# hamza1030/stereo_matching_cuda

Hardware: AMD Instinct MI355X
Metric: disparity MPix/s (stereo pair -> L+R disparity + occlusion-filled map) (higher is better)
Workload: dtype f32; 1 GPU; kitti 1242x375 D=192 seeded synthetic pair (seed 20150101); width=1242, height=375, disparities=192, slices_in_flight=192, walker_launches_per_call=1

## Files before the change

stereo_matching_cuda_amd/csrc/smx_agg_v5.hip:

```cpp
#include <stdlib.h>
#include <string.h>

#include <type_traits>

#include "smx_agg_dev.h"
#include "smx_agg_v5.h"
#include "smx_v5_diag.h"

namespace smx {
namespace v5 {
using namespace aggdev;

constexpr int R = 9, HW = 2 * R + 1;
constexpr int SWU = HW * L;
constexpr int SW = (SWU + 3) / 4 * 4;
static_assert(OWS == HW * (L - 1) && SWU == OWS + HW && CPW * L <= 64 && CPW * NS1 >= HW, "strip geometry");
constexpr int RD = 20;
static_assert(RD % BH == 0 && RD >= HW + 1, "ring");
static_assert(L == 9, "the shipped form: seven combs of nine lanes per comb wave");
constexpr int NX = 2;
constexpr int NWAVE = 2 * NS1 + NX, NT = 64 * NWAVE;
constexpr int WPE = 4;
constexpr int NT1 = 3, NT2 = 2;
enum Role { ROLE_S1 = 0, ROLE_S2 = 1, ROLE_SCAN = 2, ROLE_COST = 3 };
// ... 21 lines not shown
    return d;
}

__device__ __forceinline__ f2 div_ca(f2 x, f2 ca) {
    f2 q, e, m;
    asm("v_pk_mul_f32 %0, %1, %2 op_sel_hi:[1,0]" : "=v"(q) : "v"(x), "v"(ca));
    asm("v_pk_fma_f32 %0, %1, %2, %3 op_sel:[0,1,0] op_sel_hi:[1,1,1] neg_lo:[1,0,0] neg_hi:[1,0,0]" : "=v"(e) : "v"(q), "v"(ca), "v"(x));
    asm("v_pk_fma_f32 %0, %1, %2, %3 op_sel_hi:[1,0,1]" : "=v"(m) : "v"(e), "v"(ca), "v"(q));
    return m;
}

__device__ __forceinline__ f2 div_ca_q(f2 x, f2 ca) { f2 q; asm("v_pk_mul_f32 %0, %1, %2 op_sel_hi:[1,0]" : "=v"(q) : "v"(x), "v"(ca)); return q; }
__device__ __forceinline__ f2 div_ca_e(f2 q, f2 x, f2 ca) {
    f2 e;
    asm("v_pk_fma_f32 %0, %1, %2, %3 op_sel:[0,1,0] op_sel_hi:[1,1,1] neg_lo:[1,0,0] neg_hi:[1,0,0]" : "=v"(e) : "v"(q), "v"(ca), "v"(x));
    return e;
}
__device__ __forceinline__ f2 div_ca_m(f2 e, f2 q, f2 ca) { f2 m; asm("v_pk_fma_f32 %0, %1, %2, %3 op_sel_hi:[1,0,1]" : "=v"(m) : "v"(e), "v"(ca), "v"(q)); return m; }

__device__ __forceinline__ unsigned cost_trunc_h2(unsigned q1, unsigned q2, unsigned th2) {
    unsigned d;
    asm("v_pk_add_f16 %0, %1, %2 neg_lo:[0,1] neg_hi:[0,1]" : "=v"(d) : "v"(q1), "v"(q2));
    d &= 0x7fff7fffu;
    asm("v_pk_min_f16 %0, %1, %2" : "=v"(d) : "v"(d), "s"(th2));
    return d;
}
__device__ __forceinline__ float mix_mul_lo(unsigned h2, float s) {
    float r;
    asm("v_fma_mix_f32 %0, %1, %2, 0 op_sel_hi:[1,0,0]" : "=v"(r) : "v"(h2), "s"(s));
    return r;
}
__device__ __forceinline__ float mix_mul_hi(unsigned h2, float s) {
    float r;
    asm("v_fma_mix_f32 %0, %1, %2, 0 op_sel:[1,0,0] op_sel_hi:[1,0,0]" : "=v"(r) : "v"(h2), "s"(s));
    return r;
}
__device__ __forceinline__ float mix_mul_lo_v(unsigned h2, float v) {
    float r;
    asm("v_fma_mix_f32 %0, %1, %2, 0 op_sel_hi:[1,0,0]" : "=v"(r) : "v"(h2), "v"(v));
    return r;
}

__device__ __forceinline__ f2 tile_rd(const float* p) { return (f2){p[0], p[P1]}; }
__device__ __forceinline__ void tile_wr(float* p, f2 v) { p[0] = v.x; p[P1] = v.y; }

template <int FASTK, int QP>
__global__ __launch_bounds__(NT, WPE) void k_v5_walk(Args A) {
    constexpr bool QPERM = QP != 0;
    __shared__ __attribute__((aligned(16))) float tile1[NT1][TILE_F];
    __shared__ __attribute__((aligned(16))) float tile2s[NT2][TILE_F];
    __shared__ float cin1s[2][BH][2];
    __shared__ float rcp_s[RCP_N];
    __shared__ int s_queue[4];
    __shared__ unsigned s_peekn;
    __shared__ unsigned s_seen;
    __shared__ unsigned s_peek[2];
    __shared__ unsigned s_x1;

    const int lane = threadIdx.x & 63;
    const int wave = __builtin_amdgcn_readfirstlane(threadIdx.x >> 6);
    const int tid = 64 * wave + lane;
    const int w = A.w, h = A.h, K = A.K, NI = A.NI, nsv = A.nsv;
    const CostConst cc = A.cc;
    const f2 NZ2 = {-0.0f, -0.0f};
    if (tid < RCP_N) rcp_s[tid] = kRcp.v[tid];

    const bool st2w = wave >= NS1 && wave < 2 * NS1;
    auto comb_il = [&]() { return opaque(lane) % L; };
    auto comb_rho = [&]() {
        const int l = opaque(lane), c = l / L;
        return c < CPW ? CPW * (wave - (st2w ? NS1 : 0)) + c : HW;
    };
    auto comb_jt = [&]() {
        const int rho = comb_rho(), il = comb_il();
        return rho < HW ? HW * il + rho : 0;
    };
    constexpr int NQROW = SW / 4;
    constexpr int NCT = 64;
    constexpr int NRB = 4;
    constexpr int NRBC = 4;
    static_assert(2 * NRBC >= (BH * (SW / 4) + 63) / 64, "two batches");
    constexpr int NCT2 = 0;
    constexpr int NQT = BH * NQROW;
    constexpr int NRQ = (NQT - NCT2 + NCT - 1) / NCT;

    if (tid == 0) {
        s_queue[0] = (int)__hip_atomic_fetch_add((gu32*)A.ticket, 1u, __ATOMIC_RELAXED, __HIP_MEMORY_SCOPE_AGENT);
        s_x1 = 0u; s_peek[0] = 0u; s_peek[1] = 0u; s_peekn = 0u;
    }
    const int P = A.P, q_last = (h + 37) / 10;
    const unsigned fgw4 = ((unsigned)w + 2u * PADX) * 4u, w4 = (unsigned)w * 4u;
    const rsrc_t r_fix = mk_rsrc(A.fix, A.fix_bytes);
    const unsigned recb = (unsigned)(NI + 2) * REC_U * 16u;
    const rsrc_t r_hand = mk_rsrc(A.hand, (size_t)2 * nsv * recb);
    {
        auto item_body = [&](auto ROLEc) {
        constexpr int ROLE = decltype(ROLEc)::value;
        constexpr bool ST2 = ROLE == ROLE_S2, COMB = ROLE <= ROLE_S2;
        int item = 0, k = 0, sv = 0, view = 0, slice = 0, d = 0;
        int base1 = 0;
        int base2 = 0;
        bool pred = false, succ = false;
        bool xedge = false;
        unsigned* myflag = A.flags;
        int o_fg1 = 0, o_fg2 = 0, o_g1p = 0, o_i2p = 0, o_i2b = 0, o_in = 0, o_out = 0;
        rsrc_t r_q = r_fix;
        int q_pitch = 0, q_row0 = 0;
        auto decode = [&](int it) {
            item = it;
            k = it / nsv;
            sv = it - k * nsv;
            view = sv / A.nslices;
            slice = sv - view * A.nslices;
            base1 = OWS * k - 1;
            base2 = OWS * k - R - 1;
            pred = k > 0; succ = k + 1 < K;
            d = A.d0[view] + slice;
            myflag = A.flags + (size_t)sv * K + k;
            o_fg1 = (int)A.o_fg[view]; o_fg2 = (int)A.o_fg[view ^ 1];
            o_g1p = (int)(A.o_g1p[view] + (unsigned)k * (unsigned)(5 * NI) * (CLP * 16u));
            o_i2p = (int)(A.o_i2p[view] + (unsigned)k * (unsigned)NI * (CLP * 16u));
            o_i2b = (int)(A.o_i2p[view] + (unsigned)K * (unsigned)NI * (CLP * 16u) + (unsigned)k * (unsigned)NI * (CLP * 4u));
            o_in = (int)((((unsigned)(k - 1) & 1u) * (unsigned)nsv + (unsigned)sv) * recb);
            o_out = (int)((((unsigned)k & 1u) * (unsigned)nsv + (unsigned)sv) * recb);
            r_q = mk_rsrc(A.q[view] + (size_t)slice * A.q_plane, A.q_plane * 4);
            q_pitch = QPERM ? OWS * 8 : (int)w4; q_row0 = QPERM ? k * ((h + 1) / 2) * (OWS * 8) : 0;
            xedge = base1 < 0 || base1 + SW > w;
        };
        float* tile2 = tile2s[0];
        float (*cin1)[2] = cin1s[0];
        const int jt = comb_jt();
        int xw = 1;
        float rcp_i = 1.0f;
        unsigned vo = OOB;
        unsigned vg = 0;
        bool col_ok = false;
        f2 ca_i = {1.0f, 1.0f};
        uint64_t okmask = 0;
        const bool il0 = comb_il() == 0;
        int jw = 0;
        static_assert(SW + 16 <= P1 && P1 + SW + 16 <= RS, "padding columns behind both planes of a tile row");
        auto lane_consts = [&]() {
            const int il = comb_il();
            const int xo = (ST2 ? base2 - R : base2) + jt;
            col_ok = comb_rho() < HW && xo >= 0 && xo < w && (!ST2 || il >= 1);
            xw = col_ok ? min(w - 1, xo + R) - max(-1, xo - R - 1) : 1;
            rcp_i = rcp_s[HW * xw];
            {
                const int cl = 64 * (wave - (st2w ? NS1 : 0)) + lane;
                vg = (unsigned)cl * (ST2 ? 4u : 16u);
                vo = !col_ok ? OOB : (QPERM ? (unsigned)(k + 1 < K ? (L - 1) * comb_rho() + il - 1 : HW * (il - 1) + comb_rho()) * 8u : (unsigned)xo * 4u);
            }
            ca_i = (f2){rcp_i, (float)(HW * xw)};
            okmask = __builtin_amdgcn_ballot_w64(col_ok);
            jw = (comb_rho() < HW && !(pred && comb_il() == 0)) ? jt : SW + (lane & 15);
        };

        f2 ring[COMB ? RD : 1];
        auto ring_reset = [&]() {
#pragma unroll
            for (int s = 0; s < (COMB ? RD : 1); ++s) ring[s] = (f2){0.0f, 0.0f};
            if constexpr (COMB) ring[ST2 ? 10 : RD - 1] = NZ2;
        };
        ring_reset();
        f4 gr[ROLE == ROLE_S1 ? 2 : 1];
        for (int e = 0; e < (ROLE == ROLE_S1 ? 2 : 1); ++e) gr[e] = (f4){0, 0, 0, 0};
        unsigned gI[ST2 ? BH / 2 : 1];
        f2 r2[ST2 ? BH : 1];
#pragma unroll
        for (int t = 0; t < (ST2 ? BH : 1); ++t) r2[t] = NZ2;
        f4 hreg = {0, 0, 0, 0};
        bool have_pref = false;
        unsigned seen = 0;

        auto cost_unit = [&](int r, int& row, int& col, bool& on) {
            const int u = NCT2 + r * NCT + opaque(lane);
            on = u < NQT;
            const int uc = min(u, NQT - 1);
            row = uc / NQROW;
            col = (uc - row * NQROW) * 4;
        };
        constexpr int CWN = ROLE == ROLE_COST ? NRQ : 1;
        unsigned cw_a1[CWN], cw_a2[CWN], cw_t[CWN], cw_rowb[CWN], cw_m[CWN];
        for (int r = 0; r < CWN; ++r) { cw_a1[r] = 0u; cw_a2[r] = 0u; cw_t[r] = 0u; cw_rowb[r] = 0u; cw_m[r] = 0u; }
        auto cost_consts = [&]() {
          if constexpr (ROLE == ROLE_COST) {
#pragma unroll
            for (int r = 0; r < NRQ; ++r) {
                int row, col; bool on;
                cost_unit(r, row, col, on);
                const unsigned rowb = (unsigned)row * fgw4;
                cw_rowb[r] = (unsigned)opaque((int)rowb);
                cw_a1[r] = (unsigned)opaque((int)((unsigned)(min(max(base1 + col, -PADX), w) + PADX) * 4u + rowb));
                cw_a2[r] = A.src_cost ? (unsigned)opaque((row * w + base1 + col) * 4)
                                      : (unsigned)opaque((int)((unsigned)(min(max(base1 + col + d, -PADX), w) + PADX) * 4u + rowb));
                cw_t[r] = (unsigned)opaque((int)(on ? (unsigned)(row * RS + col) * 4u : (unsigned)SW * 4u));
                unsigned m = 0;
#pragma unroll
                for (int j = 0; j < 4; ++j) m |= (base1 + col + j >= 0 && base1 + col + j < w) ? 1u << j : 0u;
                cw_m[r] = (unsigned)opaque((int)(m | ((unsigned)row << 8)));
            }
          }
        };
        rsrc_t r_c = r_fix;
        unsigned c_max = 0u, c_min1 = 0xffffffffu;
        const unsigned plane4 = (unsigned)(A.cost_plane * 4);
        auto cost_verdict = [&]() {
            if constexpr (ROLE == ROLE_COST) {
                if (A.src_cost && __builtin_amdgcn_ballot_w64(c_max > 0x5d800000u || c_min1 < 0x21800000u - 1u) != 0 && lane == 0)
                    flag_store(A.bad, 1u);
                c_max = 0u; c_min1 = 0xffffffffu;
            }
        };
        auto cost_rsrc = [&]() {
            if constexpr (ROLE == ROLE_COST) {
                if (A.src_cost) r_c = mk_rsrc(A.cost[view] + (size_t)slice * A.cost_plane, A.cost_plane * 4);
            }
        };
        auto cost_lin = [&](int ib, int r, int& linc4, int& sh) {
            const int row = (int)(cw_m[r] >> 8);
            const int e = max(0, BH * ib + row - (h - 1));
            const int lin4 = (int)cw_a2[r] + (BH * ib - e) * (int)w4;
            linc4 = min(max(lin4, 0), (int)plane4 - 16);
            sh = (lin4 - linc4) >> 2;
        };
        u4 cw_ra[CWN], cw_rb[CWN];
// ... 72 lines not shown
                    }
                }
#pragma unroll
                for (int j = 0; j < 4; ++j) ip[j] = mix_mul_lo_v(q1[j], pp[j]);
                if constexpr (EDGE) {
                    const bool rowok = bandb + cw_rowb[r] <= ymaxb;
#pragma unroll
                    for (int j = 0; j < 4; ++j)
                        if (!(rowok && (((cw_m[r] & 0xffu) >> j) & 1u) != 0u)) { pp[j] = -0.0f; ip[j] = -0.0f; }
                }
                *(f4*)(dstb + cw_t[r]) = pp;
                *(f4*)(dstb + cw_t[r] + P1 * 4) = ip;
            }
        };
        auto eval_band_p = [&](int ib, float* dst) {
            static_assert(2 * NRB >= CWN, "two batches");
            auto run = [&](auto EDGEc, auto SRCc) {
                constexpr int NB = decltype(SRCc)::value ? NRBC : NRB;
                cw_issue(ib, std::integral_constant<int, 0>{}, EDGEc, SRCc);
                cw_finish(ib, dst, std::integral_constant<int, 0>{}, EDGEc, SRCc);
                if constexpr (NB < CWN) {
                    cw_issue(ib, std::integral_constant<int, NB>{}, EDGEc, SRCc);
                    cw_finish(ib, dst, std::integral_constant<int, NB>{}, EDGEc, SRCc);
                }
            };
            const bool edge = xedge || BH * ib + BH > h;
            if (A.src_cost) {
                if (edge) run(std::true_type{}, std::true_type{}); else run(std::false_type{}, std::true_type{});
            } else if (edge) run(std::true_type{}, std::false_type{});
            else { V5_MARK("cost begin"); run(std::false_type{}, std::false_type{}); V5_MARK("cost end"); }
        };
        static_assert(BH == 10, "five row pairs per band");
        auto g1_load = [&](int P, auto Sc) {
            if constexpr (ROLE == ROLE_S1) {
                const int Pc = __builtin_amdgcn_readfirstlane(min(max(P, 0), 5 * NI - 1));
                const unsigned vgl = (unsigned)(64 * wave + opaque(lane)) * 16u;
                gr[decltype(Sc)::value] = __builtin_bit_cast(f4, __builtin_amdgcn_raw_buffer_load_b128(r_fix, (int)vgl, o_g1p + Pc * (CLP * 16), 0));
            }
        };
        auto issue_guid = [&](int ib, int yq0) {
            const int ibc = __builtin_amdgcn_readfirstlane(min(max(ib, 0), NI - 1));
            if constexpr (ST2) {
                const u4 a = __builtin_bit_cast(u4, __builtin_amdgcn_raw_buffer_load_b128(r_fix, (int)(vg * 4u), o_i2p + ibc * (CLP * 16), 0));
                gI[0] = a.x; gI[1] = a.y; gI[2] = a.z; gI[3] = a.w;
                gI[4] = ldu(r_fix, vg, o_i2b + ibc * (CLP * 4));
            }
        };

        auto hu_idx = [&]() { return ST2 ? opaque(tid) - 64 * NS1 : opaque(tid); };
        auto fetch_rec = [&](int rec) {
            const int hq = hu_idx();
            hreg = ld16_sc1(r_hand, (unsigned)(o_in + rec * REC_U * 16) + (hq >= 0 && hq < REC_U ? (unsigned)hq * 16u : 0u));
        };
        auto spin_pred = [&](unsigned need) {
            const uint64_t t0 = __builtin_amdgcn_s_memrealtime();
            for (;;) {
                const unsigned f = flag_load(myflag - 1);
                if (f >= need) { s_seen = f; break; }
                __builtin_amdgcn_s_sleep(4);
                if (__builtin_amdgcn_s_memrealtime() - t0 > 200000000ull || flag_load(A.status) != 0u) {
                    flag_store(A.status, 1u + (unsigned)item);
                    s_seen = FLAG_DONE;
                    break;
                }
            }
        };

        auto rowscans = [&](int i1, int i2, float* t1p, float* t2p, float (*cinp)[2], bool pred1, bool pred2) {
            const int sc_l = lane & 31, sc_st = lane >> 5, sc_row = sc_l % BH, sc_comp = sc_l / BH;
            const bool sc_on = sc_l < 2 * BH;
            const int y = sc_st == 0 ? BH * i1 + sc_row : BH * i2 - R + sc_row;
            const bool act = sc_on && y >= 0 && y < h && (sc_st == 0 ? i1 >= 0 : i2 >= 0);
            if (!act) return;
            float* const row = (sc_st == 0 ? t1p : t2p) + sc_row * RS + sc_comp * P1;
            const bool keep = sc_st == 1 && pred2;
            float acc = (sc_st == 0 && pred1) ? cinp[sc_row][sc_comp] : -0.0f;
            f4* const r4 = (f4*)row;
            constexpr int NG = SW / 4;
            constexpr int PF = 4;
            f4 v[PF];
#pragma unroll
            for (int g = 0; g < PF; ++g) v[g] = r4[g];
            f4 xo[2] = {{0, 0, 0, 0}, {0, 0, 0, 0}};
#pragma unroll
            for (int g = 0; g < NG; ++g) {
                const f4 in = v[g % PF];
                if (g + PF < NG) v[g % PF] = r4[g + PF];
                f4& x = xo[g & 1];
                acc = in.x + acc; x.x = acc;
                acc = in.y + acc; x.y = acc;
                acc = in.z + acc; x.z = acc;
                if (g == 4 && keep) acc = in.z;
                acc = in.w + acc; x.w = acc;
                if (g < 5 && keep) { x.x = in.x; x.y = in.y; x.z = in.z; if (g < 4) x.w = in.w; }
                r4[g] = x;
                asm volatile("" :: "v"(xo[(g & 1) ^ 1]));
            }
        };

        auto area_ix = [&](int y) {
            const unsigned yh = min((unsigned)(min(y + R, h - 1) - max(y - R - 1, -1)), (unsigned)HW);
            return (int)__umul24((unsigned)xw, max(yh, 1u));
        };
        auto rcp_pair = [&](int y) {
            const int a0 = area_ix(y), a1 = area_ix(y + 1);
            return (f4){rcp_s[a0], (float)a0, rcp_s[a1], (float)a1};
        };
        f4 rcb = {1.0f, 1.0f, 1.0f, 1.0f};

        unsigned x1_need = 0;
        auto wait_x1 = [&]() {
            for (unsigned spins = 0; __hip_atomic_load(&s_x1, __ATOMIC_RELAXED, __HIP_MEMORY_SCOPE_WORKGROUP) < x1_need; ++spins) {
                __builtin_amdgcn_s_sleep(1);
                if (spins > (1u << 24)) { flag_store(A.status, 1u + (unsigned)item); break; }
            }
            asm volatile("" ::: "memory");
        };
        auto rows1_pair = [&](auto N0c, auto EDGEc, auto BORDERc, auto WAITc, int i, const float* t1, f2& rv) {
            f2 caa = ca_i, cab = ca_i;
            f4 rcn = {1.0f, 1.0f, 1.0f, 1.0f};
            constexpr int N0 = decltype(N0c)::value, T0 = N0 % BH, GS = (N0 / BH + T0 / 2) & 1;
            constexpr bool BORDER = decltype(BORDERc)::value;
            constexpr bool EDGE = decltype(EDGEc)::value || BORDER;
            constexpr int SLa = N0, SLb = N0 + 1, SLPa = (N0 + RD - 1) % RD, S01a = (N0 + 1) % RD, S01b = (N0 + 2) % RD;
            const f2 rvb = tile_rd(t1 + (T0 + 1) * RS + jt);
            const f2 rvn = tile_rd(t1 + (T0 + 2 < BH ? T0 + 2 : T0 + 1) * RS + jt);
            const int ya = BH * i - R + T0;
            if constexpr (decltype(BORDERc)::value) {
                caa = (f2){rcb.x, rcb.y};
                cab = (f2){rcb.z, rcb.w};
                rcn = rcp_pair(ya + 2);
            }
            const f2 old_a = ring[S01a];
            ring[SLa] = rv + ring[SLPa];
            f2 ua = box_bottom(ring[SLa]);
            const f2 sb = rvb + ring[SLa];
            ua = ua - old_a;
            f2 ub = box_bottom(sb);
            ua = box_top(ua, old_a);
            ring[SLb] = sb;
            ub = ub - ring[S01b];
            if constexpr (EDGE) {
                const f2 u0a = ring[SLa] - old_a;
                if (il0 && k == 0) ua = u0a;
            }
            const f2 qa = div_ca_q(ua, caa);
            ub = box_top(ub, ring[S01b]);
            if constexpr (EDGE) {
                const f2 u0b = sb - ring[S01b];
                if (il0 && k == 0) ub = u0b;
            }
            const f2 qb = div_ca_q(ub, cab);
            f2 ma = qa, mb = qb;
            if constexpr (!FASTK) ma = div_ca_m(div_ca_e(qa, ua, caa), qa, caa);
            const f2 ga = {gr[GS].x, gr[GS].y}, gb = {gr[GS].z, gr[GS].w};
            const float mma = ga.x * ma.x;
            if constexpr (!FASTK) mb = div_ca_m(div_ca_e(qb, ub, cab), qb, cab);
            const float ta = ma.y - mma;
            const float mmb = gb.x * mb.x;
            const float aka = 1.0f * ta * ga.y;
            const float tb = mb.y - mmb;
            const float mb2a = 1.0f * ga.x * aka;
            const float akb = 1.0f * tb * gb.y;
            const float bka = 1.0f * ma.x - mb2a;
            const float mb2b = 1.0f * gb.x * akb;
// ... 49 lines not shown
                    tiny = !(amin >= 0x1p-100f);
                } else {
                    float m1, m2;
                    asm("v_min_f32 %0, |%1|, |%2|" : "=v"(m1) : "v"(ua.x), "v"(ua.y));
                    mb = div_ca_m(div_ca_e(qb, ub, cab), qb, cab);
                    asm("v_min_f32 %0, |%1|, |%2|" : "=v"(m2) : "v"(ub.x), "v"(ub.y));
                    tiny = (va && !(m1 >= 0x1p-100f)) || (vb && !(m2 >= 0x1p-100f));
                }
            }
            if (!FASTK && (__builtin_amdgcn_ballot_w64(tiny) & okmask) != 0) {
                asm volatile("; exact-division slow path");
                ma.x = 1.0f * ua.x / caa.y; ma.y = 1.0f * ua.y / caa.y;
                mb.x = 1.0f * ub.x / cab.y; mb.y = 1.0f * ub.y / cab.y;
            }
            const fg_t ip = __builtin_bit_cast(fg_t, gI[T0 / 2]);
            const float tqa = ma.x * (float)ip.x;
            const float tqb = mb.x * (float)ip.y;
            float qva = tqa + ma.y;
            float qvb = tqb + mb.y;
            if constexpr (QPERM) {
                if (va) __builtin_amdgcn_raw_buffer_store_b64((u2){__builtin_bit_cast(unsigned, qva), __builtin_bit_cast(unsigned, qvb)}, r_q, (int)vo, q_row0 + (yq >> 1) * q_pitch, AUX_NT);
            } else {
                if (va) __builtin_amdgcn_raw_buffer_store_b32(__builtin_bit_cast(unsigned, qva), r_q, (int)vo, q_row0 + yq * q_pitch, AUX_NT);
                if (vb) __builtin_amdgcn_raw_buffer_store_b32(__builtin_bit_cast(unsigned, qvb), r_q, (int)vo, q_row0 + (yq + 1) * q_pitch, AUX_NT);
            }
            if constexpr (BORDER) rcb = rcn;
            __builtin_amdgcn_sched_barrier(0);
        };

        auto hand_in = [&](bool halo, const f4 hreg) {
            const int hq = hu_idx();
            if (hq >= 0 && hq < NHU) {
                if (halo) {
                    const int t = hq / 10, j = (hq - 10 * t) * 2;
                    float* dst = tile2 + t * RS + j;
                    dst[0] = hreg.x;
                    dst[P1] = hreg.y;
                    if (j + 1 < HW) { dst[1] = hreg.z; dst[P1 + 1] = hreg.w; }
                }
            } else if (hq >= NHU && hq < REC_U) {
                const int tp = hq - NHU;
                cin1[2 * tp][0] = hreg.x; cin1[2 * tp][1] = hreg.y;
                cin1[2 * tp + 1][0] = hreg.z; cin1[2 * tp + 1][1] = hreg.w;
            }
        };

        float* G1[3] = {tile1[1], tile1[2], tile1[0]};
        float* G2[2] = {tile2s[0], tile2s[1]};
        float (*GC[2])[2] = {cin1s[0], cin1s[1]};
        int g = 0;
        int nf = 0;
        int slf = -2;
        bool ending = false;
        bool f_pred = false;
        bool own = false;
        constexpr int sw = 1;
        int pend_item = 0; bool pend = false;
        int sl2 = 0;
        bool b_pred = false, b_own = false;
        int nxt = 0;

        auto slot_s1 = [&](auto PARc, int sl) {
            constexpr int PAR = decltype(PARc)::value;
            [[maybe_unused]] const int i = g;
            if constexpr (ROLE == ROLE_S1) {
                fetch_rec(min(sl + 2, NI - 1));
                if (sl == -2) {
                    g1_load(0, std::integral_constant<int, 0>{});
                    g1_load(1, std::integral_constant<int, 1>{});
                }
                if (sl >= 0) {
                    const float* const t1 = G1[0];
                    f2 rv = tile_rd(t1 + jt);
                    tile2 = G2[0];
                    V5_STAMP(3);
                    if (sl == 0 && succ && tid < NCU) {
                        const float* p = t1 + 2 * tid * RS + OWS - 1;
                        st16_sc1(r_hand, (unsigned)o_out + (unsigned)(NHU + tid) * 16u, (f4){p[0], p[P1], p[RS], p[RS + P1]});
                    }
                    if (A.prio) __builtin_amdgcn_s_setprio(PRIO_S1);
                    x1_need = (unsigned)NS1 * (unsigned)(g + 1);
                    const bool border = BH * sl - R < R + 1 || BH * sl - R + BH - 1 > h - 1 - R;
                    V5_STAMP(4);
                    __builtin_amdgcn_sched_barrier(0);
#define V5_P1(TT) rows1_pair(std::integral_constant<int, BH * PAR + TT>{}, std::false_type{}, std::false_type{}, std::integral_constant<bool, TT == 0>{}, sl, t1, rv);
#define V5_P1E(TT) rows1_pair(std::integral_constant<int, BH * PAR + TT>{}, std::true_type{}, std::false_type{}, std::integral_constant<bool, TT == 0>{}, sl, t1, rv);
#define V5_P1B(TT) rows1_pair(std::integral_constant<int, BH * PAR + TT>{}, std::true_type{}, std::true_type{}, std::integral_constant<bool, TT == 0>{}, sl, t1, rv);
                    if (border) { rcb = rcp_pair(BH * sl - R); V5_P1B(0) V5_STAMP(6); V5_P1B(2) V5_STAMP(7); V5_P1B(4) V5_STAMP(8); V5_P1B(6) V5_STAMP(9); V5_P1B(8) V5_STAMP(10); }
                    else if (xedge || k == 0) { V5_P1E(0) V5_P1E(2) V5_P1E(4) V5_P1E(6) V5_P1E(8) }
                    else { V5_MARK("s1rows begin"); V5_P1(0) V5_STAMP(6); V5_P1(2) V5_STAMP(7); V5_P1(4) V5_STAMP(8); V5_P1(6) V5_STAMP(9); V5_P1(8) V5_STAMP(10); V5_MARK("s1rows end"); }
#undef V5_P1
#undef V5_P1E
#undef V5_P1B
                    __builtin_amdgcn_s_setprio(0);
                    V5_STAMP(11);
                }
            }
        };
        auto slot_s2 = [&](auto PARc, int sl) {
            constexpr int PAR = decltype(PARc)::value;
            [[maybe_unused]] const int i = g;
            if constexpr (ST2) {
                if (succ && tid == 64 * 2 * NS1 - 1) flag_store(myflag, (unsigned)sl);
                if (A.prio) __builtin_amdgcn_s_setprio(PRIO_S2HEAD);
                V5_MARK("s2head begin");
                const float* const t2 = G2[0];
#pragma unroll
                for (int t = 0; t < BH; ++t) r2[t] = tile_rd(t2 + t * RS + jt);
                const int hq = hu_idx();
                const bool rec_out = succ && hq >= 0 && hq < REC_U;
                f4 hov = {0.0f, 0.0f, 0.0f, 0.0f};
                if (rec_out) {
                    if (hq < NHU) {
                        const int t = hq / 10, j = (hq - 10 * t) * 2;
                        const float* p = t2 + t * RS + OWS + j;
                        hov = (f4){p[0], p[P1], p[1], p[P1 + 1]};
                    } else {
                        const float* p = G1[0] + 2 * (hq - NHU) * RS + OWS - 1;
                        hov = (f4){p[0], p[P1], p[RS], p[RS + P1]};
                    }
                }
                asm volatile("s_waitcnt lgkmcnt(0)" : "+v"(r2[0]), "+v"(r2[1]), "+v"(r2[2]), "+v"(r2[3]), "+v"(r2[4]), "+v"(r2[5]),
                             "+v"(r2[6]), "+v"(r2[7]), "+v"(r2[8]), "+v"(r2[9]), "+v"(hov) :: "memory");
                if (lane == 0) __hip_atomic_fetch_add(&s_x1, 1u, __ATOMIC_RELAXED, __HIP_MEMORY_SCOPE_WORKGROUP);
                if (rec_out) st16_sc1(r_hand, (unsigned)(o_out + sl * REC_U * 16) + (unsigned)hq * 16u, hov);
                if (BH * (sl - 2) - R + BH - 1 >= h) {
#pragma unroll
                    for (int t = 0; t < BH; ++t)
                        if (BH * (sl - 2) - R + t >= h) r2[t] = NZ2;
                }
                V5_MARK("s2head end");
                __builtin_amdgcn_s_setprio(0);
                V5_STAMP(3);
                V5_STAMP(4);
                bool s2_interior = false;
                if (sl >= 2) {
                    const int yq0 = BH * (sl - 2) - 2 * R;
                    const bool border = yq0 < R + 1 || yq0 + BH - 1 > h - 1 - R;
                    s2_interior = !border && sl != q_last;
                    __builtin_amdgcn_sched_barrier(0);
#define V5_P2(TT) rows2_pair(std::integral_constant<int, BH * PAR + TT>{}, std::false_type{}, sl);
#define V5_P2B(TT) rows2_pair(std::integral_constant<int, BH * PAR + TT>{}, std::true_type{}, sl);
                    if (border) { rcb = rcp_pair(yq0); V5_P2B(0) V5_STAMP(6); V5_P2B(2) V5_STAMP(7); V5_P2B(4) V5_STAMP(8); V5_P2B(6) V5_STAMP(9); V5_P2B(8) V5_STAMP(10); }
                    else { V5_MARK("s2rows begin"); V5_P2(0) V5_STAMP(6); V5_P2(2) V5_STAMP(7); V5_P2(4) V5_STAMP(8); V5_P2(6) V5_STAMP(9); V5_P2(8) V5_STAMP(10); V5_MARK("s2rows end"); }
#undef V5_P2
#undef V5_P2B
                }
                issue_guid(sl, BH * (sl - 1) - 2 * R);
                constexpr int KEEP = QPERM ? S2_KEEP - BH / 2 : S2_KEEP;
                if (s2_interior) asm volatile("s_waitcnt vmcnt(%0)" :: "n"(KEEP) : "memory"); else
                drain_vmem();
            }
        };

        auto iter = [&](auto PARc) -> bool {
            wg_barrier();
            [[maybe_unused]] const int i = g;
            V5_STAMP(0); V5_STAMP(1); V5_STAMP(2);
            if constexpr (ROLE >= ROLE_SCAN) { V5_STAMP(3); V5_STAMP(4); }
            if (slf == -2) {
                const int it = s_queue[nf & 3];
                ending = it >= A.nitems;
                if (ending && nf == 0) return true;
                f_pred = !ending && it / nsv > 0;
                seen = nf > 0 ? s_peekn : 0u;
                if constexpr (ROLE == ROLE_COST) {
                    if (own) cost_verdict();
                    own = !ending;
                    if (own) { decode(it); cost_consts(); cost_rsrc(); }
                } else if constexpr (ROLE == ROLE_S1) {
                    own = !ending;
                    if (own) {
                        decode(it); lane_consts(); ring_reset();
                        gr[0] = (f4){0, 0, 0, 0}; gr[1] = (f4){0, 0, 0, 0};
                    }
                } else if constexpr (ROLE == ROLE_SCAN) {
                    b_pred = pred; b_own = own;
                    own = !ending;
                    if (own) decode(it);
                } else {
                    pend_item = it; pend = !ending;
                }
            } else {
                seen = max(seen, s_peek[g & 1]);
            }
            if constexpr (ST2) {
                if (own && sl2 == q_last + 1 && succ && tid == 64 * 2 * NS1 - 1) flag_store(myflag, FLAG_DONE);
                if (slf == sw) {
                    own = pend;
                    sl2 = sw;
                    if (own) {
                        decode(pend_item); lane_consts(); ring_reset();
#pragma unroll
                        for (int t = 0; t < BH; ++t) r2[t] = NZ2;
                    }
                }
            }
            if constexpr (ROLE == ROLE_SCAN) {
                if (A.prio) __builtin_amdgcn_s_setprio(PRIO_SCAN);
                V5_MARK("scan begin");
                const int i1 = own && slf + 1 < NI ? slf + 1 : -1;
                const int i2 = slf == -2 ? (b_own ? P - 3 : -1) : (own ? slf - 1 : -1);
                rowscans(i1, i2, G1[1], G2[1], GC[0], pred, slf == -2 ? b_pred : pred);
                V5_MARK("scan end");
                __builtin_amdgcn_s_setprio(0);
            } else if constexpr (ROLE == ROLE_COST) {
                if (lane == 63) {
                    unsigned pk = 0u;
                    if (own && pred && seen != FLAG_DONE && seen < (unsigned)(slf + 4)) pk = flag_load(myflag - 1);
                    s_peek[(g + 1) & 1] = pk;
                    if (own && slf == P - 6) {
                        nxt = (int)__hip_atomic_fetch_add((gu32*)A.ticket, 1u, __ATOMIC_RELAXED, __HIP_MEMORY_SCOPE_AGENT);
                        s_queue[(nf + 1) & 3] = nxt;
                    }
                    if (own && slf == P - 3) {
                        unsigned pn = 0u;
                        if (nxt < A.nitems) {
                            const int kn = nxt / nsv, svn = nxt - kn * nsv;
                            if (kn > 0) pn = flag_load(A.flags + (size_t)svn * K + kn - 1);
                        }
                        s_peekn = pn;
                    }
                }
                if (A.prio) __builtin_amdgcn_s_setprio(PRIO_COST);
                if (own && slf + 2 < NI) eval_band_p(slf + 2, G1[2]);
                __builtin_amdgcn_s_setprio(0);
            } else if constexpr (ROLE == ROLE_S1) {
                if (own) slot_s1(PARc, slf);
            } else {
                const int sl = sl2;
                if (own && sl >= 1 && sl <= q_last) {
                    slot_s2(PARc, sl);
                } else if (lane == 0) {
                    __hip_atomic_fetch_add(&s_x1, 1u, __ATOMIC_RELAXED, __HIP_MEMORY_SCOPE_WORKGROUP);
                }
            }
            have_pref = f_pred && (seen == FLAG_DONE || seen >= (unsigned)(slf + 3));
            if (f_pred && !have_pref && slf + 2 < NI) {
                if (tid == 0) spin_pred((unsigned)(slf + 3));
                wg_barrier();
                seen = s_seen;
                if constexpr (ROLE == ROLE_S1) {
                    const int hq = hu_idx();
                    const f4 late = ld16_sc1(r_hand, (unsigned)(o_in + min(slf + 2, NI - 1) * REC_U * 16) + (hq >= 0 && hq < REC_U ? (unsigned)hq * 16u : 0u));
                    cin1 = GC[1]; tile2 = G2[0];
                    hand_in(slf >= 0, late);
                }
            } else if constexpr (ROLE == ROLE_S1) {
                V5_MARK("s1handin begin");
                if (own && pred && slf + 2 < NI) { cin1 = GC[1]; tile2 = G2[0]; hand_in(slf >= 0, hreg); }
                V5_MARK("s1handin end");
            }
            if constexpr (ROLE == ROLE_S1) {
                g1_load(slf >= 0 ? 5 * slf + 6 : slf + 2, PARc);
                if (own && slf == 0 && succ) drain_vmem();
            }
            V5_STAMP(5);
            if (ending && slf == 1) return true;
            { float* const t = G1[0]; G1[0] = G1[1]; G1[1] = G1[2]; G1[2] = t; }
            { float* const t = G2[0]; G2[0] = G2[1]; G2[1] = t; }
            { float (*const t)[2] = GC[0]; GC[0] = GC[1]; GC[1] = t; }
            ++g;
            ++sl2;
            return false;
        };
        for (;;) {
            bool done = false;
            for (slf = -2; slf < 2 && !done; slf += 2) {
                done = iter(std::integral_constant<int, 0>{});
                if (!done) { ++slf; done = iter(std::integral_constant<int, 1>{}); --slf; }
            }
            if (done) break;
            for (slf = 2; slf <= P - 3; slf += 2) {
                (void)iter(std::integral_constant<int, 0>{});
                ++slf;
                (void)iter(std::integral_constant<int, 1>{});
                --slf;
            }
            ++nf;
        }
        if constexpr (ROLE == ROLE_COST) { if (own) cost_verdict(); }
        };
        if (wave < NS1) item_body(std::integral_constant<int, ROLE_S1>{});
        else if (wave < 2 * NS1) item_body(std::integral_constant<int, ROLE_S2>{});
        else if (wave == 2 * NS1) item_body(std::integral_constant<int, ROLE_SCAN>{});
        else item_body(std::integral_constant<int, ROLE_COST>{});
    }
}

struct PermArgs {
    const float* S0[2];
    const float* S1[2];
    f2* G[2];
    uint8_t* mean_u8[2];
    double eps;
    const fg_t* FG[2];
    f2* g1p[2];
    unsigned* i2p[2];
};
__global__ __launch_bounds__(CLP) void k_v5_perm(PermArgs pa, int w, int h, int K, int NI) {
    const int cl = threadIdx.x, cw = cl >> 6, ln = cl & 63;
    const int rho = ln / L < CPW ? CPW * cw + ln / L : HW, il = ln % L;
    const int kb = blockIdx.x / (BH / 2), j = blockIdx.x - kb * (BH / 2);
    const int k = kb / NI, ib = kb - k * NI, v = blockIdx.y;
    const int x1 = OWS * k - R - 1 + HW * il + rho;
    const int xq = x1 - R;
    const bool on1 = rho < HW && x1 >= 0 && x1 < w, on2 = rho < HW && xq >= 0 && xq < w;
    {
        const int ya = min(max(BH * ib - R + 2 * j, 0), h - 1), yb = min(max(BH * ib - R + 2 * j + 1, 0), h - 1);
        f4 g = {0.0f, 0.0f, 0.0f, 0.0f};
        if (on1) {
            const f2 a = guid_point(pa.S0[v], pa.S1[v], x1, ya, w, h, R, pa.eps);
            const f2 b = yb == ya ? a : guid_point(pa.S0[v], pa.S1[v], x1, yb, w, h, R, pa.eps);
            g = (f4){a.x, a.y, b.x, b.y};
            pa.G[v][(size_t)ya * w + x1] = a;
            pa.G[v][(size_t)yb * w + x1] = b;
            if (pa.mean_u8[v]) {
                pa.mean_u8[v][(size_t)ya * w + x1] = mean_to_u8(a.x);
                pa.mean_u8[v][(size_t)yb * w + x1] = mean_to_u8(b.x);
            }
        }
        ((f4*)pa.g1p[v])[((size_t)k * (5 * NI) + 5 * ib + j) * CLP + cl] = g;
    }
    {
        const int yp = min(max((BH * (ib - 1) - 2 * R) / 2 + j, 0), (h - 1) / 2), y = 2 * yp;
        fg_t p2 = {(_Float16)0.0f, (_Float16)0.0f};
        if (on2) {
            p2.x = pa.FG[v][(size_t)y * (w + 2 * PADX) + PADX + xq].x;
            if (y + 1 < h) p2.y = pa.FG[v][(size_t)(y + 1) * (w + 2 * PADX) + PADX + xq].x;
// ... 246 lines not shown
```

stereo_matching_cuda_amd/csrc/smx_capi.hip:

```cpp
#include <limits.h>
#include <math.h>
#include <string.h>

#include <new>
#include <string>
#include <vector>

#include "smx_agg.h"
#include "smx_agg_v4.h"
#include "smx_agg_v5.h"
#include "smx_launch.h"

namespace smx {

static thread_local std::string g_err;
static thread_local int g_timing = 0;
static thread_local int g_launches = 0;
static thread_local int g_marks_dropped = 0;
struct StageTimer {
    struct Mark { int stage; hipEvent_t ev; };
    std::vector<Mark> marks;
    std::vector<std::vector<hipEvent_t>> pool;
    std::vector<size_t> used;
    void begin() { marks.clear(); for (auto& u : used) u = 0; }
// ... 21 lines not shown
    opt.keys_fresh = g_keys_fresh != 0;
    opt.max_chunk = g_max_chunk;
    AggInfo info;
    g_launches = 0;
    const int rc = aggregate(c, forced, opt, &info);
    if (rc) return rc;
    g_last_path = info.path;
    g_launches = info.launches;
    if (info.path != 1) g_last_info = info;
    return SMX_OK;
}

void stage_mark(int stage, hipStream_t st) {
    if (!g_timing) return;
    if (stage == ST_BEGIN && g_timing == 1) { g_timer.begin(); g_marks_dropped = 0; }
    if (g_timer.marks.size() >= 32768) { ++g_marks_dropped; return; }
    hipEvent_t e = g_timer.get();
    if (!e || hipEventRecord(e, st) != hipSuccess) return;
    g_timer.marks.push_back({stage, e});
}

int fail(int code, const char* fmt, ...) {
    char buf[512];
    va_list ap;
    va_start(ap, fmt);
    vsnprintf(buf, sizeof(buf), fmt, ap);
    va_end(ap);
    g_err = buf;
    return code;
}

struct DevBuf {
    void* p = nullptr;
    ~DevBuf() { if (p) (void)hipFree(p); }
    hipError_t alloc(size_t bytes) { return hipMalloc(&p, bytes ? bytes : 1); }
    template <class T> T* as() { return (T*)p; }
};

}

using namespace smx;

extern "C" {

void smx_default_params(smx_params* p) {
    if (!p) return;
    p->r_w = 0.299; p->g_w = 0.587; p->b_w = 0.0721;
    p->alpha = 0.9; p->th_color = 7; p->th_grad = 2;
    p->radius = 9; p->eps = 6.5025; p->d_lr = 0;
}

const char* smx_last_error(void) { return g_err.c_str(); }

const char* smx_version(void) { return "smx-hip gfx950 0.11 (sub-pixel disparity from the winner's neighbouring costs: smx_dev_subpixel_pair; weighted-median refinement of the filled map: smx_weighted_median; comb walker: items pipelined across tickets, q scratch in row pairs, cost volumes on the comb walker; WTA winner in the float domain; guidance in three launches; two 512-thread workgroups per CU)"; }

int smx_device_count(void) {
    int n = 0;
    if (hipGetDeviceCount(&n) != hipSuccess) return 0;
    return n;
}

int64_t smx_pack_key(float cost, uint32_t slice) { return pack_key(cost, slice); }
void smx_unpack_key(int64_t key, float* cost, uint32_t* slice) {
    float c; uint32_t s;
    unpack_key(key, &c, &s);
    if (cost) *cost = c;
    if (slice) *slice = s;
}

int smx_set_timing(int mode) {
    if (mode < 0 || mode > 2) return fail(SMX_E_ARG, "smx_set_timing: mode must be 0, 1 or 2");
    g_timing = mode;
    g_timer.begin();
    g_marks_dropped = 0;
    return SMX_OK;
}

int smx_stage_times(smx_stage_ms* out) {
    SMX_ARG(out);
    memset(out, 0, sizeof(*out));
    if (g_timer.marks.size() < 2) return fail(SMX_E_ARG, "smx_stage_times: no timed call recorded (smx_set_timing(1) first)");
    SMX_HIP(hipEventSynchronize(g_timer.marks.back().ev));
    float acc[ST_COUNT] = {0};
    int calls = g_timer.marks.front().stage == ST_BEGIN ? 1 : 0;
    for (size_t i = 1; i < g_timer.marks.size(); ++i) {
        if (g_timer.marks[i].stage == ST_BEGIN) { ++calls; continue; }
        float t = 0;
        SMX_HIP(hipEventElapsedTime(&t, g_timer.marks[i - 1].ev, g_timer.marks[i].ev));
        acc[g_timer.marks[i].stage] += t;
    }
    out->calls = calls;
    out->dropped = g_marks_dropped;
    out->upload = acc[ST_UPLOAD]; out->guidance = acc[ST_GUIDANCE]; out->aggregation = acc[ST_WALK];
    out->wta = acc[ST_WTA]; out->finish = acc[ST_FINISH]; out->download = acc[ST_DOWNLOAD];
    out->total = out->upload + out->guidance + out->aggregation + out->wta + out->finish + out->download;
    return SMX_OK;
}

int smx_last_agg_ms(float* ms, int* launches) {
    smx_stage_ms t;
    int rc = smx_stage_times(&t);
    if (rc) return rc;
    if (ms) *ms = t.guidance + t.aggregation + t.wta;
    if (launches) *launches = g_launches;
    return SMX_OK;
}

// ... 874 lines not shown
```

Baseline: 591.3 MPix/s.

## Replace per-slot workgroup barriers with LDS sequence counters between walker roles

The comb walker's roles (S1, S2, scan, cost) now hand LDS buffers to each other through per-role sequence counters, waited on with ds_read and bumped with a single-lane ds_add. The full workgroup barrier now runs only in the item-change slots. Predecessor-flag spinning moves from a tid-0 spin plus barrier into S1 itself, and the cost wave's flag peeking is removed. The aim is to let waves run ahead of each other without lockstep barriers, at the cost of more complex ordering that could deadlock or race if a counter dependency is missing.

```diff
diff --git a/stereo_matching_cuda_amd/csrc/smx_agg_v5.hip b/stereo_matching_cuda_amd/csrc/smx_agg_v5.hip
--- a/stereo_matching_cuda_amd/csrc/smx_agg_v5.hip
+++ b/stereo_matching_cuda_amd/csrc/smx_agg_v5.hip
@@ -97,12 +97,10 @@
     __shared__ float cin1s[2][BH][2];
     __shared__ float rcp_s[RCP_N];
     __shared__ int s_queue[4];
-    __shared__ unsigned s_peekn;
-    __shared__ unsigned s_seen;
-    __shared__ unsigned s_peek[2];
-    __shared__ unsigned s_x1;
-
-    const int lane = threadIdx.x & 63;
+    enum { C_COST = 0, C_SCAN, C_S1, C_X1, C_REC, C_N };
+    __shared__ __attribute__((aligned(16))) unsigned s_cnt[C_N][4];
+
+    const int lane = (int)__builtin_amdgcn_mbcnt_hi(~0u, __builtin_amdgcn_mbcnt_lo(~0u, 0u));
     const int wave = __builtin_amdgcn_readfirstlane(threadIdx.x >> 6);
     const int tid = 64 * wave + lane;
     const int w = A.w, h = A.h, K = A.K, NI = A.NI, nsv = A.nsv;
@@ -131,7 +129,8 @@
 
     if (tid == 0) {
         s_queue[0] = (int)__hip_atomic_fetch_add((gu32*)A.ticket, 1u, __ATOMIC_RELAXED, __HIP_MEMORY_SCOPE_AGENT);
-        s_x1 = 0u; s_peek[0] = 0u; s_peek[1] = 0u; s_peekn = 0u;
+        for (int c = 0; c < C_N; ++c)
+            for (int j = 0; j < 4; ++j) s_cnt[c][j] = j < (c >= C_S1 ? NS1 : 1) ? 0u : 0xffffffffu;
     }
     const int P = A.P, q_last = (h + 37) / 10;
     const unsigned fgw4 = ((unsigned)w + 2u * PADX) * 4u, w4 = (unsigned)w * 4u;
@@ -217,6 +216,8 @@
         f4 hreg = {0, 0, 0, 0};
         bool have_pref = false;
         unsigned seen = 0;
+        unsigned pk = 0;
+        unsigned pkv = 0;
 
         auto cost_unit = [&](int r, int& row, int& col, bool& on) {
             const int u = NCT2 + r * NCT + opaque(lane);
@@ -395,18 +396,45 @@
             const int hq = hu_idx();
             hreg = ld16_sc1(r_hand, (unsigned)(o_in + rec * REC_U * 16) + (hq >= 0 && hq < REC_U ? (unsigned)hq * 16u : 0u));
         };
-        auto spin_pred = [&](unsigned need) {
+        auto spin_pred = [&](unsigned need) -> unsigned {
             const uint64_t t0 = __builtin_amdgcn_s_memrealtime();
+            unsigned f;
             for (;;) {
-                const unsigned f = flag_load(myflag - 1);
-                if (f >= need) { s_seen = f; break; }
+                f = (unsigned)__builtin_amdgcn_readfirstlane((int)flag_load(myflag - 1));
+                if (f >= need) break;
                 __builtin_amdgcn_s_sleep(4);
                 if (__builtin_amdgcn_s_memrealtime() - t0 > 200000000ull || flag_load(A.status) != 0u) {
-                    flag_store(A.status, 1u + (unsigned)item);
-                    s_seen = FLAG_DONE;
+                    if (lane == 0) flag_store(A.status, 1u + (unsigned)item);
+                    f = FLAG_DONE;
                     break;
                 }
             }
+            asm volatile("" ::: "memory");
+            return f;
+        };
+        const int wir = ROLE == ROLE_S1 ? wave : ROLE == ROLE_S2 ? wave - NS1 : 0;
+        auto cnt_ld = [&](int c) {
+            u4 v;
+            asm volatile("ds_read_b128 %0, %1\n\ts_waitcnt lgkmcnt(0)" : "=v"(v) : "v"(lds_off(&s_cnt[c][0])) : "memory");
+            return (unsigned)__builtin_amdgcn_readfirstlane((int)min(min(v.x, v.y), v.z));
+        };
+        auto wait_ge = [&](int c, unsigned need) {
+            if (cnt_ld(c) < need) {
+                const unsigned t0 = (unsigned)__builtin_amdgcn_s_memrealtime();
+                for (unsigned spins = 1; cnt_ld(c) < need; ++spins) {
+                    __builtin_amdgcn_s_sleep(1);
+                    if ((spins & 1023u) == 0u && (unsigned)__builtin_amdgcn_s_memrealtime() - t0 > 400000000u) {
+                        flag_store(A.status, 1u + (unsigned)__builtin_amdgcn_readfirstlane(item));
+                        break;
+                    }
+                }
+            }
+            asm volatile("" ::: "memory");
+        };
+        auto bump = [&](int c) {
+            uint64_t ex;
+            asm volatile("s_waitcnt lgkmcnt(0)\n\ts_mov_b64 %0, exec\n\ts_mov_b64 exec, 1\n\tds_add_u32 %1, %2\n\ts_mov_b64 exec, %0"
+                         : "=&s"(ex) : "v"(lds_off(&s_cnt[c][wir])), "v"(1u) : "memory");
         };
 
         auto rowscans = [&](int i1, int i2, float* t1p, float* t2p, float (*cinp)[2], bool pred1, bool pred2) {
@@ -453,7 +481,7 @@
 
         unsigned x1_need = 0;
         auto wait_x1 = [&]() {
-            for (unsigned spins = 0; __hip_atomic_load(&s_x1, __ATOMIC_RELAXED, __HIP_MEMORY_SCOPE_WORKGROUP) < x1_need; ++spins) {
+            for (unsigned spins = 0; cnt_ld(C_X1) < x1_need; ++spins) {
                 __builtin_amdgcn_s_sleep(1);
                 if (spins > (1u << 24)) { flag_store(A.status, 1u + (unsigned)item); break; }
             }
@@ -609,13 +637,11 @@
         int nf = 0;
         int slf = -2;
         bool ending = false;
-        bool f_pred = false;
         bool own = false;
         constexpr int sw = 1;
         int pend_item = 0; bool pend = false;
         int sl2 = 0;
         bool b_pred = false, b_own = false;
-        int nxt = 0;
 
         auto slot_s1 = [&](auto PARc, int sl) {
             constexpr int PAR = decltype(PARc)::value;
@@ -626,6 +652,8 @@
                     g1_load(0, std::integral_constant<int, 0>{});
                     g1_load(1, std::integral_constant<int, 1>{});
                 }
+                wait_ge(C_SCAN, (unsigned)g);
+                pk = (unsigned)__builtin_amdgcn_readfirstlane((int)pkv);
                 if (sl >= 0) {
                     const float* const t1 = G1[0];
                     f2 rv = tile_rd(t1 + jt);
@@ -636,7 +664,7 @@
                         st16_sc1(r_hand, (unsigned)o_out + (unsigned)(NHU + tid) * 16u, (f4){p[0], p[P1], p[RS], p[RS + P1]});
                     }
                     if (A.prio) __builtin_amdgcn_s_setprio(PRIO_S1);
-                    x1_need = (unsigned)NS1 * (unsigned)(g + 1);
+                    x1_need = (unsigned)(g + 1);
                     const bool border = BH * sl - R < R + 1 || BH * sl - R + BH - 1 > h - 1 - R;
                     V5_STAMP(4);
                     __builtin_amdgcn_sched_barrier(0);
@@ -658,6 +686,7 @@
             constexpr int PAR = decltype(PARc)::value;
             [[maybe_unused]] const int i = g;
             if constexpr (ST2) {
+                wait_ge(C_SCAN, (unsigned)g);
                 if (succ && tid == 64 * 2 * NS1 - 1) flag_store(myflag, (unsigned)sl);
                 if (A.prio) __builtin_amdgcn_s_setprio(PRIO_S2HEAD);
                 V5_MARK("s2head begin");
@@ -679,7 +708,7 @@
                 }
                 asm volatile("s_waitcnt lgkmcnt(0)" : "+v"(r2[0]), "+v"(r2[1]), "+v"(r2[2]), "+v"(r2[3]), "+v"(r2[4]), "+v"(r2[5]),
                              "+v"(r2[6]), "+v"(r2[7]), "+v"(r2[8]), "+v"(r2[9]), "+v"(hov) :: "memory");
-                if (lane == 0) __hip_atomic_fetch_add(&s_x1, 1u, __ATOMIC_RELAXED, __HIP_MEMORY_SCOPE_WORKGROUP);
+                if (lane == 0) __hip_atomic_fetch_add(&s_cnt[C_X1][wir], 1u, __ATOMIC_RELAXED, __HIP_MEMORY_SCOPE_WORKGROUP);
                 if (rec_out) st16_sc1(r_hand, (unsigned)(o_out + sl * REC_U * 16) + (unsigned)hq * 16u, hov);
                 if (BH * (sl - 2) - R + BH - 1 >= h) {
 #pragma unroll
@@ -710,17 +739,16 @@
             }
         };
 
-        auto iter = [&](auto PARc) -> bool {
-            wg_barrier();
+        auto iter = [&](auto PARc, auto BARc) -> bool {
+            if constexpr (decltype(BARc)::value) wg_barrier();
             [[maybe_unused]] const int i = g;
             V5_STAMP(0); V5_STAMP(1); V5_STAMP(2);
             if constexpr (ROLE >= ROLE_SCAN) { V5_STAMP(3); V5_STAMP(4); }
             if (slf == -2) {
-                const int it = s_queue[nf & 3];
+                const int it = __builtin_amdgcn_readfirstlane(s_queue[nf & 3]);
                 ending = it >= A.nitems;
                 if (ending && nf == 0) return true;
-                f_pred = !ending && it / nsv > 0;
-                seen = nf > 0 ? s_peekn : 0u;
+                seen = 0u;
                 if constexpr (ROLE == ROLE_COST) {
                     if (own) cost_verdict();
                     own = !ending;
@@ -738,10 +766,9 @@
                 } else {
                     pend_item = it; pend = !ending;
                 }
-            } else {
-                seen = max(seen, s_peek[g & 1]);
             }
             if constexpr (ST2) {
+                if (own && succ && wave == 2 * NS1 - 1) wait_ge(C_REC, (unsigned)g);
                 if (own && sl2 == q_last + 1 && succ && tid == 64 * 2 * NS1 - 1) flag_store(myflag, FLAG_DONE);
                 if (slf == sw) {
                     own = pend;
@@ -758,59 +785,52 @@
                 V5_MARK("scan begin");
                 const int i1 = own && slf + 1 < NI ? slf + 1 : -1;
                 const int i2 = slf == -2 ? (b_own ? P - 3 : -1) : (own ? slf - 1 : -1);
+                wait_ge(C_COST, (unsigned)g);
+                wait_ge(C_S1, (unsigned)g);
                 rowscans(i1, i2, G1[1], G2[1], GC[0], pred, slf == -2 ? b_pred : pred);
                 V5_MARK("scan end");
                 __builtin_amdgcn_s_setprio(0);
+                bump(C_SCAN);
             } else if constexpr (ROLE == ROLE_COST) {
-                if (lane == 63) {
-                    unsigned pk = 0u;
-                    if (own && pred && seen != FLAG_DONE && seen < (unsigned)(slf + 4)) pk = flag_load(myflag - 1);
-                    s_peek[(g + 1) & 1] = pk;
-                    if (own && slf == P - 6) {
-                        nxt = (int)__hip_atomic_fetch_add((gu32*)A.ticket, 1u, __ATOMIC_RELAXED, __HIP_MEMORY_SCOPE_AGENT);
-                        s_queue[(nf + 1) & 3] = nxt;
-                    }
-                    if (own && slf == P - 3) {
-                        unsigned pn = 0u;
-                        if (nxt < A.nitems) {
-                            const int kn = nxt / nsv, svn = nxt - kn * nsv;
-                            if (kn > 0) pn = flag_load(A.flags + (size_t)svn * K + kn - 1);
-                        }
-                        s_peekn = pn;
-                    }
-                }
+                wait_ge(C_S1, (unsigned)g);
+                wait_ge(C_X1, (unsigned)g);
+                if (lane == 63 && own && slf == P - 6)
+                    s_queue[(nf + 1) & 3] = (int)__hip_atomic_fetch_add((gu32*)A.ticket, 1u, __ATOMIC_RELAXED, __HIP_MEMORY_SCOPE_AGENT);
                 if (A.prio) __builtin_amdgcn_s_setprio(PRIO_COST);
                 if (own && slf + 2 < NI) eval_band_p(slf + 2, G1[2]);
                 __builtin_amdgcn_s_setprio(0);
+                bump(C_COST);
             } else if constexpr (ROLE == ROLE_S1) {
+                pk = 0u;
+                pkv = flag_load(own && pred ? myflag - 1 : A.flags);
                 if (own) slot_s1(PARc, slf);
             } else {
                 const int sl = sl2;
                 if (own && sl >= 1 && sl <= q_last) {
                     slot_s2(PARc, sl);
                 } else if (lane == 0) {
-                    __hip_atomic_fetch_add(&s_x1, 1u, __ATOMIC_RELAXED, __HIP_MEMORY_SCOPE_WORKGROUP);
-                }
-            }
-            have_pref = f_pred && (seen == FLAG_DONE || seen >= (unsigned)(slf + 3));
-            if (f_pred && !have_pref && slf + 2 < NI) {
-                if (tid == 0) spin_pred((unsigned)(slf + 3));
-                wg_barrier();
-                seen = s_seen;
-                if constexpr (ROLE == ROLE_S1) {
+                    __hip_atomic_fetch_add(&s_cnt[C_X1][wir], 1u, __ATOMIC_RELAXED, __HIP_MEMORY_SCOPE_WORKGROUP);
+                }
+                bump(C_REC);
+            }
+            if constexpr (ROLE == ROLE_S1) {
+                const bool f_pred = own && pred;
+                have_pref = f_pred && (seen == FLAG_DONE || seen >= (unsigned)(slf + 3));
+                if (f_pred && !have_pref && slf + 2 < NI) {
+                    seen = spin_pred((unsigned)(slf + 3));
                     const int hq = hu_idx();
                     const f4 late = ld16_sc1(r_hand, (unsigned)(o_in + min(slf + 2, NI - 1) * REC_U * 16) + (hq >= 0 && hq < REC_U ? (unsigned)hq * 16u : 0u));
                     cin1 = GC[1]; tile2 = G2[0];
                     hand_in(slf >= 0, late);
-                }
-            } else if constexpr (ROLE == ROLE_S1) {
-                V5_MARK("s1handin begin");
-                if (own && pred && slf + 2 < NI) { cin1 = GC[1]; tile2 = G2[0]; hand_in(slf >= 0, hreg); }
-                V5_MARK("s1handin end");
-            }
-            if constexpr (ROLE == ROLE_S1) {
+                } else {
+                    V5_MARK("s1handin begin");
+                    if (f_pred && slf + 2 < NI) { cin1 = GC[1]; tile2 = G2[0]; hand_in(slf >= 0, hreg); }
+                    V5_MARK("s1handin end");
+                }
+                seen = max(seen, pk);
                 g1_load(slf >= 0 ? 5 * slf + 6 : slf + 2, PARc);
                 if (own && slf == 0 && succ) drain_vmem();
+                bump(C_S1);
             }
             V5_STAMP(5);
             if (ending && slf == 1) return true;
@@ -824,14 +844,14 @@
         for (;;) {
             bool done = false;
             for (slf = -2; slf < 2 && !done; slf += 2) {
-                done = iter(std::integral_constant<int, 0>{});
-                if (!done) { ++slf; done = iter(std::integral_constant<int, 1>{}); --slf; }
+                done = iter(std::integral_constant<int, 0>{}, std::true_type{});
+                if (!done) { ++slf; done = iter(std::integral_constant<int, 1>{}, std::true_type{}); --slf; }
             }
             if (done) break;
             for (slf = 2; slf <= P - 3; slf += 2) {
-                (void)iter(std::integral_constant<int, 0>{});
+                (void)iter(std::integral_constant<int, 0>{}, std::false_type{});
                 ++slf;
-                (void)iter(std::integral_constant<int, 1>{});
+                (void)iter(std::integral_constant<int, 1>{}, std::false_type{});
                 --slf;
             }
             ++nf;
diff --git a/stereo_matching_cuda_amd/csrc/smx_capi.hip b/stereo_matching_cuda_amd/csrc/smx_capi.hip
--- a/stereo_matching_cuda_amd/csrc/smx_capi.hip
+++ b/stereo_matching_cuda_amd/csrc/smx_capi.hip
@@ -97,7 +97,7 @@
 
 const char* smx_last_error(void) { return g_err.c_str(); }
 
-const char* smx_version(void) { return "smx-hip gfx950 0.11 (sub-pixel disparity from the winner's neighbouring costs: smx_dev_subpixel_pair; weighted-median refinement of the filled map: smx_weighted_median; comb walker: items pipelined across tickets, q scratch in row pairs, cost volumes on the comb walker; WTA winner in the float domain; guidance in three launches; two 512-thread workgroups per CU)"; }
+const char* smx_version(void) { return "smx-hip gfx950 0.12 (comb walker: the roles hand their LDS buffers over through sequence counters, the slot barrier only in the item-change slots); since 0.11 (sub-pixel disparity from the winner's neighbouring costs: smx_dev_subpixel_pair; weighted-median refinement of the filled map: smx_weighted_median; comb walker: items pipelined across tickets, q scratch in row pairs, cost volumes on the comb walker; WTA winner in the float domain; guidance in three launches; two 512-thread workgroups per CU)"; }
 
 int smx_device_count(void) {
     int n = 0;
```

New measurement: 569.2 MPix/s. 0.963x the previous value.
